# awsaf49/vip-cup-2022

Measured on AMD Instinct MI355X. Metric: images/sec (200x200, full ensemble), higher is better.
Workload: dtype f16; 1 GPU; ensemble8; precision=fast, distinct_images=5120, global_batch=256, parallelism=image-parallel dp1, one all-gather of scores, member_streams=3

## Files before the change

### vip-cup-2022_amd/csrc/conv_igemm.hip

```cpp
#include "common.hpp"
#include <stdlib.h>
#include <type_traits>

#ifndef VIP_GEMM_H2
#define VIP_GEMM_H2 0
#endif

#ifndef VIP_MFMA_PRIO
#define VIP_MFMA_PRIO 1
#endif
#ifndef VIP_MFMA_PRIO_TILE
#define VIP_MFMA_PRIO_TILE 1
#endif

namespace {

constexpr bool H2 = VIP_GEMM_H2;
__device__ __forceinline__ int h2_pos(int c) { return H2 ? (((c & 1) << 2) | (c >> 1)) : c; }
constexpr unsigned OOB2 = 0xFFFFFFE0u;
constexpr int ESZ = H2 ? 4 : 2;

struct ConvArgs {
    const f16* x;
    const f16* w;
    const float* bias;
    const f16* res;
    f16* y;
    int H, W, Ho, Wo;
    int Cin_g, Cout_g;
    int kh, kw, sh, sw, pt, pl;
    int ldx, ldy, ldr, ldw;
    int cin_off, cout_off, res_off;
    int M, K;
    long x_span_bytes;
    long y_span_bytes, res_span_bytes;
    int bias_elems;
    int act_pre, act_post;
    int m_blocks, n_blocks;
    const f16* w_lo;
    const f16* gate;
    int y_lo_off;
    int gate_hw;
    float out_scale;
    int* status;
    const float* ln_g;
    const float* ln_b;
    float ln_eps;
};

enum Family { PW_GEMM, ROWS_GEMM, GEMM8P, PWX, PWK_DIRECT, PWK_GEMM, IM2COL, CONV_IGEMM };
struct Plan {
    Family family;
    int mode;
    int ng, pt, wn, ks, ksc, bm, bn;
    bool gated, hilo, ln, xsplit, pipe;
    bool pf2;
    int m_blocks, n_blocks;
    int n_chunks, nb_ch, lds_stride;
};

template <int... Vs, class F>
int with_const(int v, F&& f) {
    int st = VIP_ERR_UNSUPPORTED;
    if (!((v == Vs && ((st = f(std::integral_constant<int, Vs>{})), true)) || ...)) vip_set_error("vip_conv2d_nhwc_f16: no instantiation for %d", v);
    return st;
}

inline int device_cus() {
    static const int cus = [] {
        hipDeviceProp_t pr;
        int dev = 0;
        return (hipGetDevice(&dev) == hipSuccess && hipGetDeviceProperties(&pr, dev) == hipSuccess && pr.multiProcessorCount > 0)
                   ? pr.multiProcessorCount : 256;
    }();
    return cus;
}

template <int ACT, bool RES, int POST>
__device__ __forceinline__ void h2_store8(const ConvArgs& a, const f32x4& q0, const f32x4& q1, unsigned off, unsigned roff,
                                          const __amdgpu_buffer_rsrc_t& rb_res, const __amdgpu_buffer_rsrc_t& rb_y) {
    f32x2 p[4] = {{q0[0], q0[1]}, {q0[2], q0[3]}, {q1[0], q1[1]}, {q1[2], q1[3]}};
#pragma unroll
    for (int e = 0; e < 4; ++e) p[e] = vip_act2<ACT>(p[e] * a.out_scale);
    if constexpr (RES) {
        const uint4 rh = __builtin_bit_cast(uint4, __builtin_amdgcn_raw_buffer_load_b128(rb_res, roff, 0, 0));
        const uint4 rl = __builtin_bit_cast(uint4, __builtin_amdgcn_raw_buffer_load_b128(rb_res, roff + 16u, 0, 0));
        const unsigned rhw[4] = {rh.x, rh.y, rh.z, rh.w}, rlw[4] = {rl.x, rl.y, rl.z, rl.w};
#pragma unroll
        for (int e = 0; e < 4; ++e) {
            float px = p[e].x, py = p[e].y;
            asm("v_fma_mix_f32 %0, %1, 1.0, %0 op_sel_hi:[1,0,0]" : "+v"(px) : "v"(rhw[e]));
            asm("v_fma_mix_f32 %0, %1, 1.0, %0 op_sel:[1,0,0] op_sel_hi:[1,0,0]" : "+v"(py) : "v"(rhw[e]));
            asm("v_fma_mix_f32 %0, %1, 1.0, %0 op_sel_hi:[1,0,0]" : "+v"(px) : "v"(rlw[e]));
            asm("v_fma_mix_f32 %0, %1, 1.0, %0 op_sel:[1,0,0] op_sel_hi:[1,0,0]" : "+v"(py) : "v"(rlw[e]));
            p[e] = (f32x2){px, py};
        }
    }
    if constexpr (POST == 1) {
#pragma unroll
        for (int e = 0; e < 4; ++e) p[e] = (f32x2){fmaxf(p[e].x, 0.f), fmaxf(p[e].y, 0.f)};
    } else if constexpr (POST == 2) {
#pragma unroll
        for (int e = 0; e < 4; ++e) p[e] = (f32x2){vip_act_strict(p[e].x, a.act_post), vip_act_strict(p[e].y, a.act_post)};
    }
    typedef unsigned short u16x2 __attribute__((ext_vector_type(2)));
    unsigned hw[4], lw[4];
    u16x2 mx = {0, 0};
#pragma unroll
    for (int e = 0; e < 4; ++e) {
        hw[e] = __builtin_bit_cast(unsigned, __builtin_convertvector(p[e], f16x2));
        const float px = p[e].x, py = p[e].y;
        asm("v_fma_mixlo_f16 %0, %1, -1.0, %2 op_sel_hi:[1,0,0]" : "=v"(lw[e]) : "v"(hw[e]), "v"(px));
        asm("v_fma_mixhi_f16 %0, %1, -1.0, %2 op_sel:[1,0,0] op_sel_hi:[1,0,0]" : "+v"(lw[e]) : "v"(hw[e]), "v"(py));
        mx = __builtin_elementwise_max(mx, __builtin_bit_cast(u16x2, hw[e] & 0x7FFF7FFFu));
    }
    typedef __attribute__((__vector_size__(4 * sizeof(unsigned)))) unsigned u32x4;
    const u32x4 oh = {hw[0], hw[1], hw[2], hw[3]}, ol = {lw[0], lw[1], lw[2], lw[3]};
    __builtin_amdgcn_raw_buffer_store_b128(oh, rb_y, off, 0, 0);
    __builtin_amdgcn_raw_buffer_store_b128(ol, rb_y, off + 16u, 0, 0);
    if (a.status && off != OOB2 && (mx.x >= 0x7C00 || mx.y >= 0x7C00)) *a.status = VIP_H2_OVERFLOW;
}

__device__ __forceinline__ int swz_x(int row, int chunk) { return row * 128 + ((chunk ^ (row & 7)) << 4); }
__device__ __forceinline__ int swz_w(int row, int chunk) {
    const int key = (((row >> 3) & 3) << 1) | ((row >> 1) & 1);
    return row * 128 + ((chunk ^ key) << 4);
}

template <int ACT>
__device__ __forceinline__ float act_t(float v) {
    if constexpr (ACT == VIP_ACT_RELU) return v > 0.f ? v : 0.f;
    else if constexpr (ACT == VIP_ACT_SILU) return v * vip_sigmoid(v);
    else if constexpr (ACT == VIP_ACT_GELU) return 0.5f * v * (1.f + vip_erf(v * 0.70710678118654752f));
    else if constexpr (ACT == VIP_ACT_SIGMOID) return vip_sigmoid(v);
    else return v;
}

template <int MT, int ACT>
__device__ __forceinline__ void epilogue(const ConvArgs& a, f32x4 (&acc)[MT][4], int m_base, int n_first, int group) {
// ... 163 lines not shown
        char* sa = smem + buf * STAGE_BYTES;
        char* sb = sa + A_BYTES;
#pragma unroll
        for (int i = 0; i < A_IT; ++i) *reinterpret_cast<uint4*>(sa + swz_x(row0 + 32 * i, h2_pos(chunk))) = ra[i];
#pragma unroll
        for (int i = 0; i < B_IT; ++i) *reinterpret_cast<uint4*>(sb + swz_w(row0 + 32 * i, h2_pos(chunk))) = rb[i];
    };

    const int wave_m0 = (wave / WAVES_N) * WTM;
    const int wave_n0 = (wave % WAVES_N) * 64;
    const int l15 = lane & 15, lq = lane >> 4;
    const int wrow_base = wave_n0 + (l15 >> 2) * 8 + (l15 & 3);
    const int xrow_base = wave_m0 + l15;

    f32x4 acc[MT][4];
#pragma unroll
    for (int mt = 0; mt < MT; ++mt)
#pragma unroll
        for (int nt = 0; nt < 4; ++nt) acc[mt][nt] = (f32x4){0.f, 0.f, 0.f, 0.f};

    const int nk = (a.K + 63) >> 6;
    load_tiles(0);
    store_tiles(0);
    __syncthreads();

    for (int kt = 0; kt < nk; ++kt) {
        const int buf = kt & 1;
        if (kt + 1 < nk) load_tiles(kt + 1);
        const char* sa = smem + buf * STAGE_BYTES;
        const char* sb = sa + A_BYTES;
#pragma unroll
        for (int ks = 0; ks < 2; ++ks) {
            const int ch = ks * 4 + lq;
            U4H8 wf[4], xf[MT];
#pragma unroll
            for (int nt = 0; nt < 4; ++nt) wf[nt].u = *reinterpret_cast<const uint4*>(sb + swz_w(wrow_base + (nt >> 1) * 32 + (nt & 1) * 4, ch));
#pragma unroll
            for (int mt = 0; mt < MT; ++mt) xf[mt].u = *reinterpret_cast<const uint4*>(sa + swz_x(xrow_base + mt * 16, ch));
            if constexpr (H2) {
                U4H8 wl[4];
                if (ks == 0) {
#pragma unroll
                    for (int nt = 0; nt < 4; ++nt) wl[nt].u = *reinterpret_cast<const uint4*>(sb + swz_w(wrow_base + (nt >> 1) * 32 + (nt & 1) * 4, 4 + lq));
                } else {
#pragma unroll
                    for (int nt = 0; nt < 4; ++nt) wf[nt].u = *reinterpret_cast<const uint4*>(sb + swz_w(wrow_base + (nt >> 1) * 32 + (nt & 1) * 4, lq));
                }
                if (VIP_MFMA_PRIO_TILE) __builtin_amdgcn_s_setprio(1);
#pragma unroll
                for (int mt = 0; mt < MT; ++mt)
#pragma unroll
                    for (int nt = 0; nt < 4; ++nt) {
                        if (ks == 0) acc[mt][nt] = __builtin_amdgcn_mfma_f32_16x16x32_f16(wl[nt].h, xf[mt].h, acc[mt][nt], 0, 0, 0);
                        acc[mt][nt] = __builtin_amdgcn_mfma_f32_16x16x32_f16(wf[nt].h, xf[mt].h, acc[mt][nt], 0, 0, 0);
                    }
                if (VIP_MFMA_PRIO_TILE) __builtin_amdgcn_s_setprio(0);
                continue;
            }
            if (VIP_MFMA_PRIO_TILE) __builtin_amdgcn_s_setprio(1);
#pragma unroll
            for (int mt = 0; mt < MT; ++mt)
#pragma unroll
                for (int nt = 0; nt < 4; ++nt)
                    acc[mt][nt] = __builtin_amdgcn_mfma_f32_16x16x32_f16(wf[nt].h, xf[mt].h, acc[mt][nt], 0, 0, 0);
            if (VIP_MFMA_PRIO_TILE) __builtin_amdgcn_s_setprio(0);
        }
        if (kt + 1 < nk) store_tiles(buf ^ 1);
        __syncthreads();
    }

    const int m_base = m0 + wave_m0 + l15;
    const int n_first = n0 + wave_n0 + lq * 8;
    switch (a.act_pre) {
        case VIP_ACT_RELU: epilogue<MT, VIP_ACT_RELU>(a, acc, m_base, n_first, group); break;
        case VIP_ACT_SILU: epilogue<MT, VIP_ACT_SILU>(a, acc, m_base, n_first, group); break;
        case VIP_ACT_GELU: epilogue<MT, VIP_ACT_GELU>(a, acc, m_base, n_first, group); break;
        case VIP_ACT_SIGMOID: epilogue<MT, VIP_ACT_SIGMOID>(a, acc, m_base, n_first, group); break;
        default: epilogue<MT, VIP_ACT_NONE>(a, acc, m_base, n_first, group); break;
    }
}

template <int PT, int ACT, bool RES, bool POST_RELU>
__device__ __forceinline__ void pw_epilogue(const ConvArgs& a, f32x4 (&acc)[PT][4], int m_base, int n_first,
                                            const __amdgpu_buffer_rsrc_t& rb_res, const __amdgpu_buffer_rsrc_t& rb_y) {
    constexpr unsigned OOB = 0xFFFFFFF0u;
    if constexpr (H2) {
#pragma unroll
        for (int p = 0; p < PT; ++p) {
            const int m = m_base + p * 16;
#pragma unroll
            for (int h = 0; h < 2; ++h) {
                const int n = n_first + h * 32;
                const bool ok = (m < a.M) & (n < a.Cout_g);
                const unsigned off = ok ? (unsigned)(((long)m * a.ldy + a.cout_off + n) * 4) : OOB2;
                const unsigned roff = (RES && ok) ? (unsigned)(((long)m * a.ldr + a.res_off + n) * 4) : OOB2;
                h2_store8<ACT, RES, POST_RELU ? 1 : 0>(a, acc[p][h * 2], acc[p][h * 2 + 1], off, roff, rb_res, rb_y);
            }
        }
        return;
    }
#pragma unroll
    for (int p = 0; p < PT; ++p) {
        const int m = m_base + p * 16;
#pragma unroll
        for (int h = 0; h < 2; ++h) {
            const int n = n_first + h * 32;
            const bool ok = (m < a.M) & (n < a.Cout_g);
            U4H8 r;
            if constexpr (RES)
                r.u = __builtin_bit_cast(uint4, __builtin_amdgcn_raw_buffer_load_b128(
                                                    rb_res, ok ? ((unsigned)m * (unsigned)a.ldr + (unsigned)(a.res_off + n)) * 2u : OOB, 0, 0));
            U4H8 o;
#pragma unroll
            for (int j = 0; j < 8; j += 2) {
                const f32x4 av = acc[p][h * 2 + (j >> 2)];
                f32x2 t = vip_act2<ACT>((f32x2){av[j & 3], av[(j & 3) + 1]});
                if constexpr (RES) t = t + (f32x2){(float)r.e[j], (float)r.e[j + 1]};
                if constexpr (POST_RELU) t = (f32x2){fmaxf(t.x, 0.f), fmaxf(t.y, 0.f)};
                o.e[j] = (f16)t.x;
                o.e[j + 1] = (f16)t.y;
            }
            __builtin_amdgcn_raw_buffer_store_b128(
                __builtin_bit_cast(__attribute__((__vector_size__(4 * sizeof(unsigned)))) unsigned, o.u), rb_y,
                ok ? ((unsigned)m * (unsigned)a.ldy + (unsigned)(a.cout_off + n)) * 2u : OOB, 0, 0);
        }
    }
}

template <int KS, int PT, bool PRE, bool HILO>
__global__ __launch_bounds__(256, 2) void pw_gemm_kernel(ConvArgs a, int nb_ch, int lds_stride, int n_tiles, int mode) {
    extern __shared__ __attribute__((aligned(16))) char smem[];
    const int tid = threadIdx.x, lane = tid & 63, wave = tid >> 6;
    const int l15 = lane & 15, lq = lane >> 4;
    const int n_chunk0 = blockIdx.y * nb_ch;
    const int nch = min(nb_ch, ((a.Cout_g - n_chunk0) + 63) & ~63);
    constexpr unsigned OOB = 0xFFFFFFF0u;
    float* bias_lds = reinterpret_cast<float*>(smem + nb_ch * lds_stride);

    {
        const __amdgpu_buffer_rsrc_t rw = __builtin_amdgcn_make_buffer_rsrc(
            (void*)a.w, 0, (unsigned)min((long)0xFFFFFFF0L, 2L * a.Cout_g * a.ldw), 0x00020000);
        const __amdgpu_buffer_rsrc_t rwl = __builtin_amdgcn_make_buffer_rsrc(
            (void*)a.w_lo, 0, HILO ? (unsigned)min((long)0xFFFFFFF0L, 2L * a.Cout_g * a.ldw) : 0u, 0x00020000);
        const int cpr = KS * 4;
        constexpr int HALVES = HILO ? 2 : 1;
        for (int i = tid; i < nch * cpr * HALVES; i += 256) {
            const int j = i / (cpr * HALVES), c2 = i - j * (cpr * HALVES);
            const int c = c2 < cpr ? c2 : c2 - cpr;
            const int t = (j >> 4) & 3, r = j & 15;
            const int ch = n_chunk0 + (j & ~63) + (t >> 1) * 32 + (r >> 2) * 8 + (t & 1) * 4 + (r & 3);
            const bool ok = (ch < a.Cout_g) & (c * 8 < a.K);
            const unsigned off = ok ? (unsigned)((ch * a.ldw + c * 8) * 2) : OOB;
            const uint4 v = __builtin_bit_cast(uint4, c2 < cpr ? __builtin_amdgcn_raw_buffer_load_b128(rw, off, 0, 0)
                                                               : __builtin_amdgcn_raw_buffer_load_b128(rwl, off, 0, 0));
            *reinterpret_cast<uint4*>(smem + j * lds_stride + (H2 ? ((c2 & ~7) | h2_pos(c2 & 7)) : c2) * 16) = v;
        }
        const __amdgpu_buffer_rsrc_t rb = __builtin_amdgcn_make_buffer_rsrc(
            (void*)a.bias, 0, a.bias ? (unsigned)(a.bias_elems * 4) : 0u, 0x00020000);
        for (int i = tid; i < nch; i += 256) {
            const int ch = n_chunk0 + i;
            bias_lds[i] = __builtin_bit_cast(float, __builtin_amdgcn_raw_buffer_load_b32(rb, ch < a.Cout_g ? (unsigned)(ch * 4) : OOB, 0, 0));
        }
    }
    __syncthreads();

    const __amdgpu_buffer_rsrc_t rx = __builtin_amdgcn_make_buffer_rsrc(
        (void*)(a.x + a.cin_off), 0, (unsigned)min((long)0xFFFFFFF0L, a.x_span_bytes - 2L * a.cin_off), 0x00020000);
    const __amdgpu_buffer_rsrc_t rb_res =
        __builtin_amdgcn_make_buffer_rsrc((void*)a.res, 0, a.res ? (unsigned)a.res_span_bytes : 0u, 0x00020000);
    const __amdgpu_buffer_rsrc_t rb_y = __builtin_amdgcn_make_buffer_rsrc((void*)a.y, 0, (unsigned)a.y_span_bytes, 0x00020000);
    const char* wl = smem + l15 * lds_stride + lq * 16;

    auto load_x = [&](int tile, U4H8 (&xf)[KS][PT]) {
        const int m0 = tile * (64 * PT) + wave * (16 * PT);
#pragma unroll
        for (int ks = 0; ks < KS; ++ks)
#pragma unroll
            for (int p = 0; p < PT; ++p) {
                const int m = m0 + p * 16 + l15, k = H2 ? (ks >> 1) * 64 + lq * 16 + (ks & 1) * 8 : ks * 32 + lq * 8;
                const bool ok = (m < a.M) & (k < a.K);
                xf[ks][p].u = __builtin_bit_cast(
                    uint4, __builtin_amdgcn_raw_buffer_load_b128(rx, ok ? (unsigned)((m * a.ldx + k) * 2) : OOB, 0, 0));
            }
    };

    U4H8 xf[KS][PT], xn[PRE ? KS : 1][PRE ? PT : 1];
    int tile = blockIdx.x;
    if (tile < n_tiles) load_x(tile, xf);
// ... 644 lines not shown
                f32x4, __builtin_amdgcn_raw_buffer_load_b128(rb_bias, n < a.Cout_g ? (unsigned)(n * 4) : OOB, 0, 0));
#pragma unroll
            for (int p = 0; p < PT; ++p) acc[g][p][nt] = bv;
        }

    load_w(0);
    load_x(xf[0][0], 0, 0);
    load_x(xf[0][1], 0, 1);
    load_x(xf[1][0], 1, 0);
    load_x(xf[1][1], 1, 1);
    store_w(0);
    __syncthreads();

    auto compute = [&](int buf, const U4H8 (&xs)[PT], int ks) {
        const char* ws = smem + buf * STAGE + l15 * ROWB + lq * 16 + ks * 64;
#pragma unroll
        for (int g = 0; g < NG; ++g) {
            U4H8 wf[4];
#pragma unroll
            for (int nt = 0; nt < 4; ++nt) wf[nt].u = *reinterpret_cast<const uint4*>(ws + (g * 64 + nt * 16) * ROWB);
            if (VIP_MFMA_PRIO) __builtin_amdgcn_s_setprio(1);
#pragma unroll
            for (int nt = 0; nt < 4; ++nt)
#pragma unroll
                for (int p = 0; p < PT; ++p)
                    acc[g][p][nt] = __builtin_amdgcn_mfma_f32_16x16x32_f16(wf[nt].h, xs[p].h, acc[g][p][nt], 0, 0, 0);
            if (VIP_MFMA_PRIO) __builtin_amdgcn_s_setprio(0);
        }
    };
#define VIP_PWK2_CHUNK(SET, KC)                               \
    {                                                         \
        const int buf = (KC) & 1;                             \
        load_w((KC) + 1);                                     \
        __builtin_amdgcn_sched_barrier(0);                    \
        compute(buf, xf[SET][0], 0);                          \
        __builtin_amdgcn_sched_barrier(0);                    \
        load_x(xf[SET][0], (KC) + 2, 0);                      \
        __builtin_amdgcn_sched_barrier(0);                    \
        compute(buf, xf[SET][1], 1);                          \
        __builtin_amdgcn_sched_barrier(0);                    \
        load_x(xf[SET][1], (KC) + 2, 1);                      \
        store_w(buf ^ 1);                                     \
        __syncthreads();                                      \
    }
    for (int kc = 0; kc < nk; kc += 2) {
        VIP_PWK2_CHUNK(0, kc)
        if (kc + 1 < nk) VIP_PWK2_CHUNK(1, kc + 1)
    }
#undef VIP_PWK2_CHUNK

    int m_base = m0 + l15, n_lane = n0 + lq * 8;
    asm volatile("" : "+v"(m_base), "+v"(n_lane));
    auto epi = [&](auto gtag) {
        constexpr int G_ = decltype(gtag)::value;
        const int n_first = n_lane + G_ * 64;
        switch (mode) {
            case 1: pw_epilogue<PT, VIP_ACT_RELU, false, false>(a, acc[G_], m_base, n_first, rb_res, rb_y); break;
            case 2: pw_epilogue<PT, VIP_ACT_SILU, false, false>(a, acc[G_], m_base, n_first, rb_res, rb_y); break;
            case 3: pw_epilogue<PT, VIP_ACT_GELU, false, false>(a, acc[G_], m_base, n_first, rb_res, rb_y); break;
            case 4: pw_epilogue<PT, VIP_ACT_SIGMOID, false, false>(a, acc[G_], m_base, n_first, rb_res, rb_y); break;
            case 5: pw_epilogue<PT, VIP_ACT_NONE, true, false>(a, acc[G_], m_base, n_first, rb_res, rb_y); break;
            case 6: pw_epilogue<PT, VIP_ACT_NONE, true, true>(a, acc[G_], m_base, n_first, rb_res, rb_y); break;
            default: pw_epilogue<PT, VIP_ACT_NONE, false, false>(a, acc[G_], m_base, n_first, rb_res, rb_y); break;
        }
    };
    epi(std::integral_constant<int, 0>{});
    if constexpr (NG > 1) epi(std::integral_constant<int, 1>{});
}

#endif

template <int NG, int WN, bool IM2COL>
__global__ __launch_bounds__(256 * WN, WN == 1 ? 2 : 1) void pwk_gemm_kernel(ConvArgs a, int mode) {
    if constexpr (IM2COL) {
        const int group = blockIdx.y;
        a.x += group * a.Cin_g;
        a.w += (size_t)group * a.Cout_g * a.ldw;
        if (a.bias) a.bias += group * a.Cout_g;
        a.bias_elems -= group * a.Cout_g;
        a.cout_off += group * a.Cout_g;
        a.res_off += group * a.Cout_g;
        a.x_span_bytes -= 2L * group * a.Cin_g;
    }
    constexpr int PT = 4, NB = 64 * NG, NBLK = NB * WN, ROWB = 160;
    constexpr int NTHR = 256 * WN;
    constexpr int STAGE = NBLK * ROWB;
    constexpr int W_IT = NBLK * 8 / NTHR;
    constexpr int X_IT = 256 * 8 / NTHR;
    constexpr int XS = 64 * ROWB;
    extern __shared__ __attribute__((aligned(16))) char smem[];
    const int tid = threadIdx.x, lane = tid & 63, wave = tid >> 6;
    const int wm = wave & 3, wn = wave >> 2;
    const int l15 = lane & 15, lq = lane >> 4;
    constexpr unsigned OOB = 0xFFFFFFF0u;

    int bid = blockIdx.x;
    {
        const int nwg = gridDim.x;
        const int q = nwg >> 3, r = nwg & 7;
        const int xcd = bid & 7, idx = bid >> 3;
        bid = (xcd < r ? xcd * (q + 1) : r * (q + 1) + (xcd - r) * q) + idx;
    }
    const int mb = bid / a.n_blocks, nb = bid - mb * a.n_blocks;
    const int mblk = mb * 256;
    const int m0 = mblk + wm * 64;
    const int nblk = nb * NBLK;
    const int n0 = nblk + wn * NB;

    const __amdgpu_buffer_rsrc_t rw = __builtin_amdgcn_make_buffer_rsrc(
        (void*)a.w, 0, (unsigned)min((long)0xFFFFFFF0L, 2L * a.Cout_g * a.ldw), 0x00020000);
    const __amdgpu_buffer_rsrc_t rx = __builtin_amdgcn_make_buffer_rsrc(
        (void*)(a.x + a.cin_off), 0, (unsigned)min((long)0xFFFFFFF0L, a.x_span_bytes - 2L * a.cin_off), 0x00020000);
    const __amdgpu_buffer_rsrc_t rb_res =
        __builtin_amdgcn_make_buffer_rsrc((void*)a.res, 0, a.res ? (unsigned)a.res_span_bytes : 0u, 0x00020000);
    const __amdgpu_buffer_rsrc_t rb_y = __builtin_amdgcn_make_buffer_rsrc((void*)a.y, 0, (unsigned)a.y_span_bytes, 0x00020000);
    const __amdgpu_buffer_rsrc_t rb_bias =
        __builtin_amdgcn_make_buffer_rsrc((void*)a.bias, 0, a.bias ? (unsigned)(a.bias_elems * 4) : 0u, 0x00020000);

    const int wc = tid & 7;
    unsigned w_off[W_IT];
    int w_lds[W_IT];
#pragma unroll
    for (int i = 0; i < W_IT; ++i) {
        const int j = (tid >> 3) + (NTHR / 8) * i;
        const int t = (j >> 4) & 3, r = j & 15;
        const int ch = nblk + (j & ~63) + (t >> 1) * 32 + (r >> 2) * 8 + (t & 1) * 4 + (r & 3);
        w_off[i] = ch < a.Cout_g ? (unsigned)((ch * a.ldw + wc * 8) * 2) : OOB;
        w_lds[i] = j * ROWB + h2_pos(wc) * 16;
    }
    constexpr int XROWS = WN == 1 ? 8 : NTHR / 8;
    const int xr = WN == 1 ? wm * 64 + (lane >> 3) : (tid >> 3);
    const int xc = tid & 7;
    char* ximg = smem + 2 * STAGE;
    const unsigned x_base = (unsigned)(((mblk + xr) * a.ldx + xc * 8) * 2);
    const unsigned x_rstep = (unsigned)(XROWS * a.ldx * 2);
    int pix0[IM2COL ? X_IT : 1], hw0[IM2COL ? X_IT : 1];
    if constexpr (IM2COL) {
#pragma unroll
        for (int i = 0; i < X_IT; ++i) {
            const int m = mblk + xr + XROWS * i;
            int hi0 = -30000, wi0 = 0, pb = 0;
            if (m < a.M) {
                const int hw = a.Ho * a.Wo;
                const int b = m / hw, rem = m - b * hw;
                const int ho = rem / a.Wo, wo = rem - ho * a.Wo;
                hi0 = ho * a.sh - a.pt;
                wi0 = wo * a.sw - a.pl;
                pb = b * a.H * a.W;
            }
            pix0[i] = pb;
            hw0[i] = hi0 * 65536 + (wi0 & 0xFFFF);
        }
    }
    const int nk = (a.K + 63) >> 6;

    uint4 wst[W_IT];
    auto load_w = [&](int kc) {
        const bool ok = kc * 64 + wc * 8 < a.K;
#pragma unroll
        for (int i = 0; i < W_IT; ++i)
            wst[i] = __builtin_bit_cast(uint4, __builtin_amdgcn_raw_buffer_load_b128(rw, ok ? w_off[i] + kc * 128 : OOB, 0, 0));
    };
    auto store_w = [&](int buf) {
#pragma unroll
        for (int i = 0; i < W_IT; ++i) *reinterpret_cast<uint4*>(smem + buf * STAGE + w_lds[i]) = wst[i];
    };
    U4H8 xst[X_IT];
    auto load_x = [&](int kc) {
        const bool kok = kc * 64 + xc * 8 < a.K;
        if constexpr (IM2COL) {
            const int k0 = kc * 64 + xc * 8;
            const int tap = k0 / a.Cin_g, c = k0 - tap * a.Cin_g;
            const int tr = tap / a.kw, ts = tap - tr * a.kw;
#pragma unroll
            for (int i = 0; i < X_IT; ++i) {
                const int hi = (hw0[i] >> 16) + tr, wi = (int)(short)(hw0[i] & 0xFFFF) + ts;
                const bool ok = kok & ((unsigned)hi < (unsigned)a.H) & ((unsigned)wi < (unsigned)a.W);
                const unsigned off = (unsigned)(((pix0[i] + hi * a.W + wi) * a.ldx + c) * 2);
                xst[i].u = __builtin_bit_cast(uint4, __builtin_amdgcn_raw_buffer_load_b128(rx, ok ? off : OOB, 0, 0));
            }
        } else {
#pragma unroll
            for (int i = 0; i < X_IT; ++i) {
                const bool ok = kok & (mblk + xr + XROWS * i < a.M);
                xst[i].u = __builtin_bit_cast(
                    uint4, __builtin_amdgcn_raw_buffer_load_b128(rx, ok ? x_base + i * x_rstep + kc * 128 : OOB, 0, 0));
            }
        }
    };
    auto store_x = [&]() {
#pragma unroll
        for (int i = 0; i < X_IT; ++i) {
            *reinterpret_cast<uint4*>(ximg + (xr + XROWS * i) * ROWB + h2_pos(xc) * 16) = xst[i].u;
        }
    };
    const char* xs = ximg + wm * XS;

    f32x4 acc[NG][PT][4];
    {
#pragma unroll
        for (int g = 0; g < NG; ++g)
#pragma unroll
            for (int nt = 0; nt < 4; ++nt) {
                const int n = n0 + g * 64 + (nt >> 1) * 32 + lq * 8 + (nt & 1) * 4;
                const f32x4 bv = __builtin_bit_cast(
                    f32x4, __builtin_amdgcn_raw_buffer_load_b128(rb_bias, n < a.Cout_g ? (unsigned)(n * 4) : OOB, 0, 0));
#pragma unroll
                for (int p = 0; p < PT; ++p) acc[g][p][nt] = bv;
            }
    }

    load_w(0);
    load_x(0);
    store_w(0);
    store_x();
    __syncthreads();

    auto compute = [&](int buf, int ks) {
        const char* ws = smem + buf * STAGE + (WN > 1 ? wn * NB * ROWB : 0) + l15 * ROWB + lq * 16 + ks * 64;
        const char* xl = xs + l15 * ROWB + lq * 16 + ks * 64;
        U4H8 xf[PT];
#pragma unroll
        for (int p = 0; p < PT; ++p) xf[p].u = *reinterpret_cast<const uint4*>(xl + p * 16 * ROWB);
#pragma unroll
        for (int g = 0; g < NG; ++g) {
            U4H8 wf[4];
            if constexpr (H2) {
                const char* wh = ws - ks * 64;
                U4H8 wl[4];
#pragma unroll
                for (int nt = 0; nt < 4; ++nt) wf[nt].u = *reinterpret_cast<const uint4*>(wh + (g * 64 + nt * 16) * ROWB);
                if (ks == 0) {
#pragma unroll
                    for (int nt = 0; nt < 4; ++nt) wl[nt].u = *reinterpret_cast<const uint4*>(wh + 64 + (g * 64 + nt * 16) * ROWB);
                }
                if (VIP_MFMA_PRIO) __builtin_amdgcn_s_setprio(1);
#pragma unroll
                for (int nt = 0; nt < 4; ++nt)
#pragma unroll
                    for (int p = 0; p < PT; ++p) {
                        if (ks == 0) acc[g][p][nt] = __builtin_amdgcn_mfma_f32_16x16x32_f16(wl[nt].h, xf[p].h, acc[g][p][nt], 0, 0, 0);
                        acc[g][p][nt] = __builtin_amdgcn_mfma_f32_16x16x32_f16(wf[nt].h, xf[p].h, acc[g][p][nt], 0, 0, 0);
                    }
                if (VIP_MFMA_PRIO) __builtin_amdgcn_s_setprio(0);
                continue;
            }
#pragma unroll
            for (int nt = 0; nt < 4; ++nt) wf[nt].u = *reinterpret_cast<const uint4*>(ws + (g * 64 + nt * 16) * ROWB);
            if (VIP_MFMA_PRIO) __builtin_amdgcn_s_setprio(1);
#pragma unroll
            for (int nt = 0; nt < 4; ++nt)
#pragma unroll
                for (int p = 0; p < PT; ++p)
                    acc[g][p][nt] = __builtin_amdgcn_mfma_f32_16x16x32_f16(wf[nt].h, xf[p].h, acc[g][p][nt], 0, 0, 0);
            if (VIP_MFMA_PRIO) __builtin_amdgcn_s_setprio(0);
        }
    };

    for (int kc = 0; kc < nk; ++kc) {
        const int buf = kc & 1;
        load_w(kc + 1);
        load_x(kc + 1);
        __builtin_amdgcn_sched_barrier(0);
        compute(buf, 0);
        compute(buf, 1);
        __builtin_amdgcn_sched_barrier(0);
        store_w(buf ^ 1);
        if constexpr (WN > 1) __syncthreads();
        store_x();
        __syncthreads();
    }

    int m_base = m0 + l15, n_lane = n0 + lq * 8;
    asm volatile("" : "+v"(m_base), "+v"(n_lane));
    auto epi = [&](auto gtag) {
        constexpr int G_ = decltype(gtag)::value;
        const int n_first = n_lane + G_ * 64;
        switch (mode) {
            case 1: pw_epilogue<PT, VIP_ACT_RELU, false, false>(a, acc[G_], m_base, n_first, rb_res, rb_y); break;
            case 2: pw_epilogue<PT, VIP_ACT_SILU, false, false>(a, acc[G_], m_base, n_first, rb_res, rb_y); break;
            case 3: pw_epilogue<PT, VIP_ACT_GELU, false, false>(a, acc[G_], m_base, n_first, rb_res, rb_y); break;
            case 4: pw_epilogue<PT, VIP_ACT_SIGMOID, false, false>(a, acc[G_], m_base, n_first, rb_res, rb_y); break;
            case 5: pw_epilogue<PT, VIP_ACT_NONE, true, false>(a, acc[G_], m_base, n_first, rb_res, rb_y); break;
            case 6: pw_epilogue<PT, VIP_ACT_NONE, true, true>(a, acc[G_], m_base, n_first, rb_res, rb_y); break;
            default: pw_epilogue<PT, VIP_ACT_NONE, false, false>(a, acc[G_], m_base, n_first, rb_res, rb_y); break;
        }
    };
    epi(std::integral_constant<int, 0>{});
    if constexpr (NG > 1) epi(std::integral_constant<int, 1>{});
}

template <int NG>
int launch_pwk_direct(const ConvArgs& a, const Plan& p, hipStream_t s) {
    auto go = [&](auto kernel) { hipLaunchKernelGGL(kernel, dim3((unsigned)(a.m_blocks * a.n_blocks)), dim3(256), 0, s, a, p.mode); };
    if (p.pt == 1) p.gated ? go(pwk_direct_kernel<NG, true, 1>) : go(pwk_direct_kernel<NG, false, 1>);
#if VIP_BUILD_EXPERIMENTS
    else if (p.pf2) go(pwk_direct2_kernel<NG>);
#endif
    else p.gated ? go(pwk_direct_kernel<NG, true, 4>) : go(pwk_direct_kernel<NG, false, 4>);
    return vip_launch_status("vip_conv2d_nhwc_f16(pwk-direct)");
}

template <int NG, int WN, bool IM2COL>
int launch_pwk(const ConvArgs& a, int mode, int groups, hipStream_t s) {
    constexpr size_t smem = (2 * 64 * NG * WN + 4 * 64) * 160;
    static bool attr_set = false;
    if (!attr_set) {
        (void)hipFuncSetAttribute(reinterpret_cast<const void*>(pwk_gemm_kernel<NG, WN, IM2COL>),
                                  hipFuncAttributeMaxDynamicSharedMemorySize, (int)smem);
        attr_set = true;
    }
    const dim3 grid((unsigned)(a.m_blocks * a.n_blocks), (unsigned)groups);
    hipLaunchKernelGGL((pwk_gemm_kernel<NG, WN, IM2COL>), grid, dim3(256 * WN), smem, s, a, mode);
    return vip_launch_status(IM2COL ? "vip_conv2d_nhwc_f16(pwk-im2col)" : "vip_conv2d_nhwc_f16(pwk)");
}

#include "gemm8p.hpp"

template <bool XSPLIT>
__global__ __launch_bounds__(256) void rows_gemm_kernel(ConvArgs a) {
    constexpr unsigned OOB = 0xFFFFFFF0u;
    __shared__ float red[3][1][16][64];
    const int tid = threadIdx.x, lane = tid & 63, wave = tid >> 6;
    const int mw = 0, kq = wave;
    const int l15 = lane & 15, lq = lane >> 4;
    const int n0 = blockIdx.x * 16;
    const int m0 = blockIdx.y * 64;
    const __amdgpu_buffer_rsrc_t rw = __builtin_amdgcn_make_buffer_rsrc(
        (void*)a.w, 0, (unsigned)min((long)0xFFFFFFF0L, 2L * a.Cout_g * a.ldw), 0x00020000);
    const __amdgpu_buffer_rsrc_t rx = __builtin_amdgcn_make_buffer_rsrc(
        (void*)(a.x + a.cin_off), 0, (unsigned)min((long)0xFFFFFFF0L, a.x_span_bytes - 2L * a.cin_off), 0x00020000);
    const unsigned w_off = (n0 + l15 < a.Cout_g) ? (unsigned)(((n0 + l15) * a.ldw + lq * (H2 ? 16 : 8)) * 2) : 0xFFFF0000u;
    unsigned x_off[4];
#pragma unroll
    for (int p = 0; p < 4; ++p) {
        const int m = m0 + p * 16 + l15;
        x_off[p] = m < a.M ? (unsigned)((m * a.ldx + lq * (H2 ? 16 : 8)) * 2) : 0xFFFF0000u;
    }
    f32x4 acc[4];
#pragma unroll
    for (int p = 0; p < 4; ++p) acc[p] = (f32x4){0.f, 0.f, 0.f, 0.f};
    const int nks = H2 ? 2 * ((a.K + 63) >> 6) : (a.K + 31) >> 5;
    const int per = ((nks + 3) / 4 + 3) & ~3;
    const int ks_lo = kq * per, ks_hi = min(nks, ks_lo + per);
    if (m0 < a.M) {
        for (int ks0 = ks_lo; ks0 < ks_hi; ks0 += 4) {
            U4H8 wf[4], xf[4][4];
#pragma unroll
            for (int u = 0; u < 4; ++u) {
                const int kst = ks0 + u;
                const bool ok = (kst < ks_hi) & ((H2 ? (kst >> 1) * 64 + lq * 16 + (kst & 1) * 8 : kst * 32 + lq * 8) < a.K);
                const unsigned kb = H2 ? (unsigned)((kst >> 1) * 128 + (kst & 1) * 16) : (unsigned)(kst * 64);
                wf[u].u = __builtin_bit_cast(uint4, __builtin_amdgcn_raw_buffer_load_b128(rw, ok ? w_off + kb : OOB, 0, 0));
#pragma unroll
                for (int p = 0; p < 4; ++p)
                    xf[u][p].u = __builtin_bit_cast(uint4, __builtin_amdgcn_raw_buffer_load_b128(rx, ok ? x_off[p] + kb : OOB, 0, 0));
            }
            if constexpr (H2) {
#pragma unroll
                for (int u = 0; u < 4; u += 2)
#pragma unroll
                    for (int p = 0; p < 4; ++p) {
                        acc[p] = __builtin_amdgcn_mfma_f32_16x16x32_f16(wf[u + 1].h, xf[u][p].h, acc[p], 0, 0, 0);
                        acc[p] = __builtin_amdgcn_mfma_f32_16x16x32_f16(wf[u].h, xf[u + 1][p].h, acc[p], 0, 0, 0);
                        acc[p] = __builtin_amdgcn_mfma_f32_16x16x32_f16(wf[u].h, xf[u][p].h, acc[p], 0, 0, 0);
                    }
                continue;
            }
// ... 130 lines not shown
    }
#endif
    plan_blocks(p, a, 64 * p.pt, 64 * p.ng);
    return VIP_OK;
}

static int plan_pwk(Plan& p, const ConvArgs& a, int ng, int wn) {
    p.family = PWK_GEMM; p.ng = ng; p.wn = wn;
    plan_blocks(p, a, 256, 64 * ng * wn);
    return VIP_OK;
}

static int plan(const ConvArgs& a, const vip_conv_desc* d, bool x_split, Plan* out) {
    Plan& p = *out = Plan{};
    const long M = a.M;
    const int cin_g = d->Cin / d->groups, cout_g = a.Cout_g;
    const bool residual = a.res, gate = a.gate, w_lo = a.w_lo;
    int mode = -1;
    if (!residual && d->act_post == VIP_ACT_NONE) mode = d->act_pre;
    else if (residual && d->act_pre == VIP_ACT_NONE && d->act_post == VIP_ACT_NONE) mode = 5;
    else if (residual && d->act_pre == VIP_ACT_NONE && d->act_post == VIP_ACT_RELU) mode = 6;
    p.mode = mode;
#if !VIP_GEMM_H2
    if (a.ln_g) {
        VIP_REQUIRE(mode >= 0 && a.ln_b && !w_lo && !gate && !a.y_lo_off && !x_split && d->groups == 1 && d->kh == 1 && d->kw == 1 && d->sh == 1 &&
                        d->sw == 1 && d->pt == 0 && d->pl == 0 && d->Ho == d->H && d->Wo == d->W && d->cin_off == 0 &&
                        vip_ln_gemm_supported((int)M, a.K, cout_g, d->act_pre) && a.x_span_bytes < 0xFFFF0000L - 2L * a.K,
                    VIP_ERR_UNSUPPORTED,
                    "vip_ln_gemm_bias_act_f16: M=%ld K=%d N=%d act=%d/%d%s not taken (vip_ln_gemm_supported; (activation) or "
                    "(residual [+ReLU]) epilogue)", M, a.K, cout_g, d->act_pre, d->act_post, residual ? " +res" : "");
        const int ksc = (a.K + 63) >> 6;
        return plan_pwx(p, a, ksc <= 2 ? 2 : ksc <= 3 ? 3 : ksc <= 4 ? 4 : 6, 2, true);
    }
#endif
    const bool short_k = a.K <= 256;
    static const int pw_mode = getenv("VIP_PW") ? atoi(getenv("VIP_PW")) : 3;
    if (pw_mode && d->groups == 1 && d->kh == 1 && d->kw == 1 && d->sh == 1 && d->sw == 1 && d->pt == 0 && d->pl == 0 &&
        d->Ho == d->H && d->Wo == d->W) {
        if (w_lo) {
            VIP_REQUIRE(mode >= 0 && short_k && !gate && !a.y_lo_off, VIP_ERR_UNSUPPORTED,
                        "vip_conv2d_hilo_nhwc_f16: 1x1 stride-1 ungrouped, K <= 256, (activation) or (residual [+ReLU]) epilogue");
            return plan_pw(p, a);
        }
        if (M <= 256 && !residual && !gate && d->act_post == VIP_ACT_NONE && d->ldy % 4 == 0 && d->cout_off % 4 == 0 &&
            a.x_span_bytes < 0xFFFF0000L - 2L * a.K && 2L * cout_g * d->ldw < 0xFFFF0000L - 2L * a.K) {
            p.family = ROWS_GEMM; p.xsplit = x_split;
            return VIP_OK;
        }
        VIP_REQUIRE(!a.y_lo_off && !x_split, VIP_ERR_UNSUPPORTED, "vip_gemm_split_f16: at most 256 rows, N %% 4 == 0");
        if (mode >= 0 && (pw_mode & 1) && short_k && M >= 65536 && !gate) return plan_pw(p, a);
        const char* g8_env = getenv("VIP_G8P_MINK");
        const int g8_min_k = g8_env ? atoi(g8_env) : 1024;
        if (mode >= 0 && g8_min_k > 0 && !gate && a.K >= g8_min_k && gemm8p_eligible(a) && cout_g % 256 == 0 &&
            (long)((M + 255) / 256) * (cout_g / 256) >= 128) {
            p.family = GEMM8P; p.pipe = a.K % 128 == 0;
            plan_blocks(p, a, 256, 256);
            return VIP_OK;
        }
        if (mode >= 0 && (pw_mode & 2) && a.x_span_bytes < 0xFFFFFFF0L) {
            static const int xl_min_k = getenv("VIP_PWK_XLK") ? atoi(getenv("VIP_PWK_XLK")) : 768;
            const char* pwx_env = getenv("VIP_PWX");
            const int pwx_on = pwx_env ? atoi(pwx_env) : 0;
            if (pwx_on && !gate && cout_g >= 256 && a.K <= (H2 ? 512 : 256) && a.K > 64 && M >= 16384 && a.x_span_bytes < 0xFFFF0000L - 2L * a.K) {
                const int ksc = (a.K + 63) >> 6;
                if (H2) {
                    if (ksc <= 4) return plan_pwx(p, a, 4, 2, false);
                    return plan_pwx(p, a, ksc <= 6 ? 6 : 8, 1, false);
                }
                return plan_pwx(p, a, ksc <= 2 ? 2 : ksc <= 3 ? 3 : 4, 2, false);
            }
            if ((a.K < xl_min_k || gate) && a.x_span_bytes < 0xFFFF0000L - 2L * a.K) return plan_pwk_direct(p, a);
            VIP_REQUIRE(!gate, VIP_ERR_UNSUPPORTED, "vip_conv2d_gated_nhwc_f16: input tensor too large (4 GB - 2K)");
            if (cout_g <= 64) return plan_pwk(p, a, 1, 1);
            static const int wn2_min_k = getenv("VIP_PWK_WN2K") ? atoi(getenv("VIP_PWK_WN2K")) : 1024;
            if (cout_g % 256 == 0 && a.K >= wn2_min_k && (long)((M + 255) / 256) * (cout_g / 256) >= 256) return plan_pwk(p, a, 2, 2);
            return plan_pwk(p, a, 2, 1);
        }
    }
    {
        static const int im2col_all = getenv("VIP_PWK_CONV") ? atoi(getenv("VIP_PWK_CONV")) : 0;
        if ((cin_g <= 16 || im2col_all > 0 || (im2col_all == 0 && M >= 32768)) && mode >= 0 && !gate && a.x_span_bytes < 0xFFFFFFF0L && d->H < 30000 &&
            d->W < 30000 && d->pt < 16 && d->pl < 16) {
            p.family = IM2COL; p.ng = cout_g <= 64 ? 1 : 2;
            plan_blocks(p, a, 256, 64 * p.ng);
            return VIP_OK;
        }
    }
    VIP_REQUIRE(!w_lo, VIP_ERR_UNSUPPORTED, "vip_conv2d_hilo_nhwc_f16: only 1x1 stride-1 ungrouped convolutions with K <= 256");
    VIP_REQUIRE(!gate, VIP_ERR_UNSUPPORTED,
                "vip_conv2d_gated_nhwc_f16: only 1x1 stride-1 ungrouped convolutions with (activation) or (residual [+ReLU]) "
                "epilogues take a gate; apply vip_scale_add_act_f16 first");
    p.family = CONV_IGEMM; p.bm = short_k ? 64 : 128; p.bn = cout_g <= 64 ? 64 : 128;
    plan_blocks(p, a, p.bm, p.bn);
    return VIP_OK;
}

static int launch(const Plan& p, ConvArgs a, int groups, hipStream_t s) {
    a.m_blocks = p.m_blocks; a.n_blocks = p.n_blocks;
    switch (p.family) {
        case PW_GEMM:
            return with_const<1, 2, 3, 4, 6, 8>(p.ks, [&](auto ks) {
                constexpr int KS = decltype(ks)::value;
                return p.hilo ? launch_pw<KS, 4, true>(a, p, s) : launch_pw<KS, 4, false>(a, p, s);
            });
        case ROWS_GEMM: return p.xsplit ? launch_rows<true>(a, s) : launch_rows<false>(a, s);
        case GEMM8P: return launch_gemm8p(a, p.mode, p.pipe, s);
        case PWX:
#if !VIP_GEMM_H2
            if (p.ln) return with_const<2, 3, 4, 6>(p.ksc, [&](auto ksc) { return launch_pwx<decltype(ksc)::value, 2, true>(a, p.mode, s); });
#endif
            if (p.pt == 2) return with_const<2, 3, 4>(p.ksc, [&](auto ksc) { return launch_pwx<decltype(ksc)::value, 2, false>(a, p.mode, s); });
            return with_const<6, 8>(p.ksc, [&](auto ksc) { return launch_pwx<decltype(ksc)::value, 1, false>(a, p.mode, s); });
        case PWK_DIRECT: return p.ng == 1 ? launch_pwk_direct<1>(a, p, s) : launch_pwk_direct<2>(a, p, s);
        case PWK_GEMM:
            if (p.ng == 1) return launch_pwk<1, 1, false>(a, p.mode, groups, s);
            return p.wn == 1 ? launch_pwk<2, 1, false>(a, p.mode, groups, s) : launch_pwk<2, 2, false>(a, p.mode, groups, s);
        case IM2COL: return p.ng == 1 ? launch_pwk<1, 1, true>(a, p.mode, groups, s) : launch_pwk<2, 1, true>(a, p.mode, groups, s);
        case CONV_IGEMM:
            if (p.bn == 64) return p.bm == 64 ? launch_igemm<64, 64>(a, groups, s) : launch_igemm<128, 64>(a, groups, s);
            return p.bm == 64 ? launch_igemm<64, 128>(a, groups, s) : launch_igemm<128, 128>(a, groups, s);
    }
    return VIP_ERR_UNSUPPORTED;
}

static int conv2d_plan(const void* x, const void* gate, int y_lo_off, const void* w, const float* bias, const void* residual, void* y,
                       const vip_conv_desc* d, const void* w_lo, bool x_split, float out_scale, int* status, const float* ln_g,
                       const float* ln_b, float ln_eps, ConvArgs* args, Plan* p) {
    VIP_REQUIRE(x && w && y && d, VIP_ERR_BAD_ARG, "vip_conv2d_nhwc_f16: null pointer");
    VIP_REQUIRE(d->B > 0 && d->H > 0 && d->W > 0 && d->Cin > 0 && d->Cout > 0 && d->kh > 0 && d->kw > 0 &&
                    d->sh > 0 && d->sw > 0 && d->Ho > 0 && d->Wo > 0 && d->groups > 0 && d->pt >= 0 && d->pl >= 0,
                VIP_ERR_BAD_ARG, "vip_conv2d_nhwc_f16: non-positive dimension");
    VIP_REQUIRE(d->Cin % d->groups == 0 && d->Cout % d->groups == 0, VIP_ERR_BAD_ARG,
                "vip_conv2d_nhwc_f16: channels (%d,%d) not divisible by groups %d", d->Cin, d->Cout, d->groups);
    const int cin_g = d->Cin / d->groups, cout_g = d->Cout / d->groups;
    VIP_REQUIRE(cin_g % 8 == 0 && cout_g % 8 == 0, VIP_ERR_ALIGNMENT,
                "vip_conv2d_nhwc_f16: Cin/groups=%d and Cout/groups=%d must be multiples of 8", cin_g, cout_g);
    VIP_REQUIRE(d->ldx % 8 == 0 && d->ldy % 8 == 0 && d->ldw % 8 == 0 && d->cin_off % 8 == 0 &&
                    d->cout_off % 8 == 0 && (!residual || (d->ldr % 8 == 0 && d->res_off % 8 == 0)),
                VIP_ERR_ALIGNMENT, "vip_conv2d_nhwc_f16: strides/offsets must be multiples of 8 halfs");
    constexpr int IN = H2 ? 2 : 1;
    VIP_REQUIRE(d->ldx >= d->cin_off + d->Cin && d->ldy >= d->cout_off + d->Cout && d->ldw >= IN * d->kh * d->kw * cin_g,
                VIP_ERR_BAD_ARG, "vip_conv2d_nhwc_f16: leading dimension smaller than the channel extent");
    VIP_REQUIRE(!H2 || (d->ldw % 16 == 0 && !w_lo && !y_lo_off && !x_split), VIP_ERR_BAD_ARG,
                "vip_conv2d_nhwc_h2: ldw must be a multiple of 16 halfs; no split variants");
    VIP_REQUIRE((unsigned)d->act_pre <= 4u && (unsigned)d->act_post <= 4u, VIP_ERR_BAD_ARG,
                "vip_conv2d_nhwc_f16: unknown activation code");
    const long M = (long)d->B * d->Ho * d->Wo;
    VIP_REQUIRE(M < (1L << 31) - 256, VIP_ERR_UNSUPPORTED, "vip_conv2d_nhwc_f16: B*Ho*Wo too large");

    ConvArgs& a = *args;
    a.x = (const f16*)x; a.w = (const f16*)w; a.bias = bias; a.res = (const f16*)residual; a.y = (f16*)y;
    a.H = d->H; a.W = d->W; a.Ho = d->Ho; a.Wo = d->Wo;
    a.Cin_g = cin_g * IN; a.Cout_g = cout_g;
    a.kh = d->kh; a.kw = d->kw; a.sh = d->sh; a.sw = d->sw; a.pt = d->pt; a.pl = d->pl;
    a.ldx = d->ldx * IN; a.ldy = d->ldy; a.ldr = d->ldr; a.ldw = d->ldw;
    a.cin_off = d->cin_off * IN; a.cout_off = d->cout_off; a.res_off = d->res_off;
    a.M = (int)M; a.K = d->kh * d->kw * cin_g * IN;
    a.x_span_bytes = 2L * IN * d->B * d->H * d->W * d->ldx;
    a.y_span_bytes = (long)ESZ * M * d->ldy;
    a.res_span_bytes = (long)ESZ * M * d->ldr;
    a.bias_elems = d->Cout;
    a.out_scale = out_scale;
    a.status = status;
    VIP_REQUIRE(a.y_span_bytes < 0xFFFFFFE0L && a.res_span_bytes < 0xFFFFFFE0L, VIP_ERR_UNSUPPORTED,
                "vip_conv2d_nhwc_f16: output or residual tensor exceeds the 4 GiB buffer-addressing range");
    VIP_REQUIRE(a.x_span_bytes < 0xFFFFFFF0L && 2L * d->Cout * d->ldw < 0xFFFFFFF0L, VIP_ERR_UNSUPPORTED,
                "vip_conv2d_nhwc_f16: input or weight tensor exceeds the 4 GiB buffer-addressing range");
    a.act_pre = d->act_pre; a.act_post = d->act_post;
    a.m_blocks = a.n_blocks = 0;
    a.w_lo = (const f16*)w_lo;
    a.gate = (const f16*)gate;
    a.gate_hw = d->Ho * d->Wo;
    a.y_lo_off = y_lo_off;
    a.ln_g = ln_g; a.ln_b = ln_b; a.ln_eps = ln_eps;
    return plan(a, d, x_split, p);
}

static int conv2d_impl(const void* x, const void* gate, int y_lo_off, const void* w, const float* bias, const void* residual, void* y,
                       const vip_conv_desc* d, void* stream, const void* w_lo = nullptr, bool x_split = false, float out_scale = 1.f,
                       int* status = nullptr, const float* ln_g = nullptr, const float* ln_b = nullptr, float ln_eps = 0.f) {
    ConvArgs a;
    Plan p;
    const int st = conv2d_plan(x, gate, y_lo_off, w, bias, residual, y, d, w_lo, x_split, out_scale, status, ln_g, ln_b, ln_eps, &a, &p);
    return st != VIP_OK ? st : launch(p, a, d->groups, (hipStream_t)stream);
}

static int kernel_query(const char* who, bool variant, const vip_conv_desc* d, int has_residual, int has_gate, int has_w_lo, char* out,
                        size_t cap) {
    VIP_REQUIRE(d && out && cap > 0, VIP_ERR_BAD_ARG, "%s: null pointer", who);
    static const char dummy[16] = {0};
    ConvArgs a;
    Plan p;
    const int st = conv2d_plan(dummy, has_gate ? dummy : nullptr, 0, dummy, nullptr, has_residual ? dummy : nullptr, const_cast<char*>(dummy), d,
                               has_w_lo ? dummy : nullptr, false, 1.f, nullptr, nullptr, nullptr, 0.f, &a, &p);
    if (st != VIP_OK) return st;
    static const char* const kernel[] = {"pw_gemm_kernel",    "rows_gemm_kernel", "gemm8p_kernel",           "pwx_kernel",
                                         "pwk_direct_kernel", "pwk_gemm_kernel",  "pwk_gemm_kernel(im2col)", "conv_igemm_kernel"};
    if (!variant) {
        snprintf(out, cap, "%s", p.family == PWX && p.ln ? "pwx_ln_kernel" : kernel[p.family]);
        return VIP_OK;
// ... 118 lines not shown
```

Before: 4722 images/sec.

## Trim dead N-tiles and simplify index math in im2col pointwise GEMM

In the im2col path of the pointwise GEMM kernel, this adds a trim mode that skips weight staging, MFMA work and epilogue stores for 32-channel halves beyond Cout. It also drops the final K-chunk's unused half. Per-row pixel offsets are computed incrementally and folded into byte offsets, and tap/channel division uses float-reciprocal division. The aim is less wasted MFMA and address arithmetic on narrow-Cout convolutions such as stems. The cost is more code paths, plus an env/legacy fallback for huge K where the float division could lose precision.

```diff
diff --git a/vip-cup-2022_amd/csrc/conv_igemm.hip b/vip-cup-2022_amd/csrc/conv_igemm.hip
--- a/vip-cup-2022_amd/csrc/conv_igemm.hip
+++ b/vip-cup-2022_amd/csrc/conv_igemm.hip
@@ -17,6 +17,14 @@
 
 constexpr bool H2 = VIP_GEMM_H2;
 __device__ __forceinline__ int h2_pos(int c) { return H2 ? (((c & 1) << 2) | (c >> 1)) : c; }
+__device__ __forceinline__ int div22(int n, int d, float rcp_d, int& rem) {
+    int q = (int)((float)n * rcp_d);
+    int r = n - __mul24(q, d);
+    if (r < 0) { --q; r += d; }
+    else if (r >= d) { ++q; r -= d; }
+    rem = r;
+    return q;
+}
 constexpr unsigned OOB2 = 0xFFFFFFE0u;
 constexpr int ESZ = H2 ? 4 : 2;
 
@@ -55,6 +63,7 @@
     int ng, pt, wn, ks, ksc, bm, bn;
     bool gated, hilo, ln, xsplit, pipe;
     bool pf2;
+    bool legacy;
     int m_blocks, n_blocks;
     int n_chunks, nb_ch, lds_stride;
 };
@@ -384,7 +393,7 @@
 
 template <int PT, int ACT, bool RES, bool POST_RELU>
 __device__ __forceinline__ void pw_epilogue(const ConvArgs& a, f32x4 (&acc)[PT][4], int m_base, int n_first,
-                                            const __amdgpu_buffer_rsrc_t& rb_res, const __amdgpu_buffer_rsrc_t& rb_y) {
+                                            const __amdgpu_buffer_rsrc_t& rb_res, const __amdgpu_buffer_rsrc_t& rb_y, int live_h = 2) {
     constexpr unsigned OOB = 0xFFFFFFF0u;
     if constexpr (H2) {
 #pragma unroll
@@ -406,6 +415,7 @@
         const int m = m_base + p * 16;
 #pragma unroll
         for (int h = 0; h < 2; ++h) {
+            if (h >= live_h) continue;
             const int n = n_first + h * 32;
             const bool ok = (m < a.M) & (n < a.Cout_g);
             U4H8 r;
@@ -1216,6 +1226,12 @@
         a.res_off += group * a.Cout_g;
         a.x_span_bytes -= 2L * group * a.Cin_g;
     }
+    constexpr bool TRIM = IM2COL && !H2 && WN == 1;
+    bool trim = false;
+    if constexpr (IM2COL) {
+        trim = TRIM && !(mode & 0x100);
+        mode &= 0xFF;
+    }
     constexpr int PT = 4, NB = 64 * NG, NBLK = NB * WN, ROWB = 160;
     constexpr int NTHR = 256 * WN;
     constexpr int STAGE = NBLK * ROWB;
@@ -1240,6 +1256,7 @@
     const int m0 = mblk + wm * 64;
     const int nblk = nb * NBLK;
     const int n0 = nblk + wn * NB;
+    const int live = trim ? min(2 * NG, (a.Cout_g - nblk + 31) >> 5) : 2 * NG;
 
     const __amdgpu_buffer_rsrc_t rw = __builtin_amdgcn_make_buffer_rsrc(
         (void*)a.w, 0, (unsigned)min((long)0xFFFFFFF0L, 2L * a.Cout_g * a.ldw), 0x00020000);
@@ -1270,23 +1287,47 @@
     const unsigned x_rstep = (unsigned)(XROWS * a.ldx * 2);
     int pix0[IM2COL ? X_IT : 1], hw0[IM2COL ? X_IT : 1];
     if constexpr (IM2COL) {
-#pragma unroll
-        for (int i = 0; i < X_IT; ++i) {
-            const int m = mblk + xr + XROWS * i;
-            int hi0 = -30000, wi0 = 0, pb = 0;
-            if (m < a.M) {
-                const int hw = a.Ho * a.Wo;
-                const int b = m / hw, rem = m - b * hw;
-                const int ho = rem / a.Wo, wo = rem - ho * a.Wo;
-                hi0 = ho * a.sh - a.pt;
-                wi0 = wo * a.sw - a.pl;
-                pb = b * a.H * a.W;
-            }
-            pix0[i] = pb;
-            hw0[i] = hi0 * 65536 + (wi0 & 0xFFFF);
+        if (TRIM && trim && a.Wo >= XROWS) {
+            const int m_first = mblk + xr, hw = a.Ho * a.Wo;
+            int b = m_first / hw;
+            const int rem = m_first - b * hw;
+            int ho = rem / a.Wo, wo = rem - ho * a.Wo;
+#pragma unroll
+            for (int i = 0; i < X_IT; ++i) {
+                const bool in = m_first + XROWS * i < a.M;
+                pix0[i] = in ? b * a.H * a.W : 0;
+                hw0[i] = (in ? ho * a.sh - a.pt : -30000) * 65536 + (in ? (wo * a.sw - a.pl) & 0xFFFF : 0);
+                wo += XROWS;
+                if (wo >= a.Wo) {
+                    wo -= a.Wo;
+                    if (++ho >= a.Ho) { ho = 0; ++b; }
+                }
+            }
+        } else {
+#pragma unroll
+            for (int i = 0; i < X_IT; ++i) {
+                const int m = mblk + xr + XROWS * i;
+                int hi0 = -30000, wi0 = 0, pb = 0;
+                if (m < a.M) {
+                    const int hw = a.Ho * a.Wo;
+                    const int b = m / hw, rem = m - b * hw;
+                    const int ho = rem / a.Wo, wo = rem - ho * a.Wo;
+                    hi0 = ho * a.sh - a.pt;
+                    wi0 = wo * a.sw - a.pl;
+                    pb = b * a.H * a.W;
+                }
+                pix0[i] = pb;
+                hw0[i] = hi0 * 65536 + (wi0 & 0xFFFF);
+            }
+        }
+        if (TRIM && trim) {
+#pragma unroll
+            for (int i = 0; i < X_IT; ++i)
+                pix0[i] = (int)((unsigned)(pix0[i] + (hw0[i] >> 16) * a.W + (int)(short)(hw0[i] & 0xFFFF)) * (unsigned)a.ldx * 2u);
         }
     }
     const int nk = (a.K + 63) >> 6;
+    const float rcp_cin = __builtin_amdgcn_rcpf((float)a.Cin_g), rcp_kw = __builtin_amdgcn_rcpf((float)a.kw);
 
     uint4 wst[W_IT];
     auto load_w = [&](int kc) {
@@ -1295,15 +1336,32 @@
         for (int i = 0; i < W_IT; ++i)
             wst[i] = __builtin_bit_cast(uint4, __builtin_amdgcn_raw_buffer_load_b128(rw, ok ? w_off[i] + kc * 128 : OOB, 0, 0));
     };
+    static_assert(!TRIM || W_IT == 2 * NG, "one weight staging pass per 32-channel half");
     auto store_w = [&](int buf) {
 #pragma unroll
-        for (int i = 0; i < W_IT; ++i) *reinterpret_cast<uint4*>(smem + buf * STAGE + w_lds[i]) = wst[i];
+        for (int i = 0; i < W_IT; ++i) {
+            if (TRIM && i >= live) continue;
+            *reinterpret_cast<uint4*>(smem + buf * STAGE + w_lds[i]) = wst[i];
+        }
     };
     U4H8 xst[X_IT];
     auto load_x = [&](int kc) {
         const bool kok = kc * 64 + xc * 8 < a.K;
         if constexpr (IM2COL) {
             const int k0 = kc * 64 + xc * 8;
+            if (TRIM && trim) {
+                int c, ts;
+                const int tap = div22(k0, a.Cin_g, rcp_cin, c);
+                const int tr = div22(tap, a.kw, rcp_kw, ts);
+                const unsigned tap_off = (unsigned)((tr * a.W + ts) * a.ldx + c) * 2u;
+#pragma unroll
+                for (int i = 0; i < X_IT; ++i) {
+                    const int hi = (hw0[i] >> 16) + tr, wi = (int)(short)(hw0[i] & 0xFFFF) + ts;
+                    const bool ok = kok & ((unsigned)hi < (unsigned)a.H) & ((unsigned)wi < (unsigned)a.W);
+                    xst[i].u = __builtin_bit_cast(uint4, __builtin_amdgcn_raw_buffer_load_b128(rx, ok ? (unsigned)pix0[i] + tap_off : OOB, 0, 0));
+                }
+                return;
+            }
             const int tap = k0 / a.Cin_g, c = k0 - tap * a.Cin_g;
             const int tr = tap / a.kw, ts = tap - tr * a.kw;
 #pragma unroll
@@ -1379,6 +1437,22 @@
                 if (VIP_MFMA_PRIO) __builtin_amdgcn_s_setprio(0);
                 continue;
             }
+            if constexpr (TRIM) {
+#pragma unroll
+                for (int h = 0; h < 2; ++h) {
+                    if (2 * g + h >= live) continue;
+#pragma unroll
+                    for (int nt = 2 * h; nt < 2 * h + 2; ++nt) wf[nt].u = *reinterpret_cast<const uint4*>(ws + (g * 64 + nt * 16) * ROWB);
+                    if (VIP_MFMA_PRIO) __builtin_amdgcn_s_setprio(1);
+#pragma unroll
+                    for (int nt = 2 * h; nt < 2 * h + 2; ++nt)
+#pragma unroll
+                        for (int p = 0; p < PT; ++p)
+                            acc[g][p][nt] = __builtin_amdgcn_mfma_f32_16x16x32_f16(wf[nt].h, xf[p].h, acc[g][p][nt], 0, 0, 0);
+                    if (VIP_MFMA_PRIO) __builtin_amdgcn_s_setprio(0);
+                }
+                continue;
+            }
 #pragma unroll
             for (int nt = 0; nt < 4; ++nt) wf[nt].u = *reinterpret_cast<const uint4*>(ws + (g * 64 + nt * 16) * ROWB);
             if (VIP_MFMA_PRIO) __builtin_amdgcn_s_setprio(1);
@@ -1391,7 +1465,8 @@
         }
     };
 
-    for (int kc = 0; kc < nk; ++kc) {
+    const int nk_loop = trim ? nk - 1 : nk;
+    for (int kc = 0; kc < nk_loop; ++kc) {
         const int buf = kc & 1;
         load_w(kc + 1);
         load_x(kc + 1);
@@ -1404,20 +1479,29 @@
         store_x();
         __syncthreads();
     }
+    if constexpr (TRIM) {
+        if (trim) {
+            const int buf = (nk - 1) & 1;
+            compute(buf, 0);
+            if (a.K - 64 * (nk - 1) > 32) compute(buf, 1);
+        }
+    }
 
     int m_base = m0 + l15, n_lane = n0 + lq * 8;
     asm volatile("" : "+v"(m_base), "+v"(n_lane));
     auto epi = [&](auto gtag) {
         constexpr int G_ = decltype(gtag)::value;
         const int n_first = n_lane + G_ * 64;
+        const int lh = TRIM ? live - 2 * G_ : 2;
+        if (lh <= 0) return;
         switch (mode) {
-            case 1: pw_epilogue<PT, VIP_ACT_RELU, false, false>(a, acc[G_], m_base, n_first, rb_res, rb_y); break;
-            case 2: pw_epilogue<PT, VIP_ACT_SILU, false, false>(a, acc[G_], m_base, n_first, rb_res, rb_y); break;
-            case 3: pw_epilogue<PT, VIP_ACT_GELU, false, false>(a, acc[G_], m_base, n_first, rb_res, rb_y); break;
-            case 4: pw_epilogue<PT, VIP_ACT_SIGMOID, false, false>(a, acc[G_], m_base, n_first, rb_res, rb_y); break;
-            case 5: pw_epilogue<PT, VIP_ACT_NONE, true, false>(a, acc[G_], m_base, n_first, rb_res, rb_y); break;
-            case 6: pw_epilogue<PT, VIP_ACT_NONE, true, true>(a, acc[G_], m_base, n_first, rb_res, rb_y); break;
-            default: pw_epilogue<PT, VIP_ACT_NONE, false, false>(a, acc[G_], m_base, n_first, rb_res, rb_y); break;
+            case 1: pw_epilogue<PT, VIP_ACT_RELU, false, false>(a, acc[G_], m_base, n_first, rb_res, rb_y, lh); break;
+            case 2: pw_epilogue<PT, VIP_ACT_SILU, false, false>(a, acc[G_], m_base, n_first, rb_res, rb_y, lh); break;
+            case 3: pw_epilogue<PT, VIP_ACT_GELU, false, false>(a, acc[G_], m_base, n_first, rb_res, rb_y, lh); break;
+            case 4: pw_epilogue<PT, VIP_ACT_SIGMOID, false, false>(a, acc[G_], m_base, n_first, rb_res, rb_y, lh); break;
+            case 5: pw_epilogue<PT, VIP_ACT_NONE, true, false>(a, acc[G_], m_base, n_first, rb_res, rb_y, lh); break;
+            case 6: pw_epilogue<PT, VIP_ACT_NONE, true, true>(a, acc[G_], m_base, n_first, rb_res, rb_y, lh); break;
+            default: pw_epilogue<PT, VIP_ACT_NONE, false, false>(a, acc[G_], m_base, n_first, rb_res, rb_y, lh); break;
         }
     };
     epi(std::integral_constant<int, 0>{});
@@ -1714,6 +1798,8 @@
         if ((cin_g <= 16 || im2col_all > 0 || (im2col_all == 0 && M >= 32768)) && mode >= 0 && !gate && a.x_span_bytes < 0xFFFFFFF0L && d->H < 30000 &&
             d->W < 30000 && d->pt < 16 && d->pl < 16) {
             p.family = IM2COL; p.ng = cout_g <= 64 ? 1 : 2;
+            const char* legacy_env = getenv("VIP_IM2COL_LEGACY");
+            p.legacy = (legacy_env && atoi(legacy_env) != 0) || a.K >= (1 << 22);
             plan_blocks(p, a, 256, 64 * p.ng);
             return VIP_OK;
         }
@@ -1747,7 +1833,10 @@
         case PWK_GEMM:
             if (p.ng == 1) return launch_pwk<1, 1, false>(a, p.mode, groups, s);
             return p.wn == 1 ? launch_pwk<2, 1, false>(a, p.mode, groups, s) : launch_pwk<2, 2, false>(a, p.mode, groups, s);
-        case IM2COL: return p.ng == 1 ? launch_pwk<1, 1, true>(a, p.mode, groups, s) : launch_pwk<2, 1, true>(a, p.mode, groups, s);
+        case IM2COL: {
+            const int mode = p.mode | (p.legacy ? 0x100 : 0);
+            return p.ng == 1 ? launch_pwk<1, 1, true>(a, mode, groups, s) : launch_pwk<2, 1, true>(a, mode, groups, s);
+        }
         case CONV_IGEMM:
             if (p.bn == 64) return p.bm == 64 ? launch_igemm<64, 64>(a, groups, s) : launch_igemm<128, 64>(a, groups, s);
             return p.bm == 64 ? launch_igemm<64, 128>(a, groups, s) : launch_igemm<128, 128>(a, groups, s);
```

New measurement: 4445 images/sec. 0.941x the previous value.
